# genome-vendor/bsmap

Measured on NVIDIA B200. Metric: wgbs_100nt_reads_mapped_per_sec, higher is better.
Workload: dtype u32

## Files before the change

### bsmap_b200/csrc/bsx_map_impl.cuh

```cuda
#include <type_traits>
#include "bsx_map.cuh"

#include "bsx_prep.cuh"

namespace {

constexpr int ROUND_HS = bsx_round_hs(MapKernel::pe, MapKernel::rrbs, MapKernel::wide);
constexpr int FW = MapKernel::wide ? 2 : 1;

enum { CT_CAND = 0, CT_PROBE, CT_OVER, CT_FULL, CT_COMMIT, CT_MAPPED, CT_LIST, CT_GATHER };
typedef uint32_t Ctr;
#define WSET(lhs, rhs) do { const auto v_ = (rhs); __syncwarp(); if (lane == 0) (lhs) = v_; __syncwarp(); } while (0)
#define CTR_ADD(C, k, v) do { const uint32_t v_ = (uint32_t)(v); if (lane == 0) (C)[k] += v_; } while (0)

__device__ __forceinline__ uint4 *plan_of(ReadSm *R, int chain, const MapArgs &A) {
    return reinterpret_cast<uint4 *>(reinterpret_cast<uint8_t *>(R) + sizeof(ReadSm)) + chain * A.chain_stride;
}
__device__ __forceinline__ uint4 *flank_of(ReadSm *R, int chain, const MapArgs &A) {
    return reinterpret_cast<uint4 *>(reinterpret_cast<uint8_t *>(R) + sizeof(ReadSm)) + A.flank_off + chain * A.chain_stride * FW;
}

__device__ __forceinline__ uint2 read_window(const ReadSm *R, int chain, int off) {
    if (off <= -16 || off >= 16 * BSX_FIXWORDS) return make_uint2(0u, 0u);
    if (off < 0) return make_uint2(R->rw[chain][0] >> (2 * -off), R->m5[chain][0] >> (2 * -off));
    const int j = off >> 4, sh = (off & 15) * 2;
    const uint32_t r1 = (j + 1 < BSX_FIXWORDS) ? R->rw[chain][j + 1] : 0u, m1 = (j + 1 < BSX_FIXWORDS) ? R->m5[chain][j + 1] : 0u;
    return make_uint2(__funnelshift_l(r1, R->rw[chain][j], sh), __funnelshift_l(m1, R->m5[chain][j], sh));
}

__device__ __forceinline__ uint32_t flank_mask(uint32_t q, uint32_t m5) { return m5 | ((m5 & ~(q & (q >> 1))) << 1); }
__device__ __forceinline__ uint32_t ctx_mm2(const uint4 f, const uint2 c) {
    const uint32_t ub = (f.x ^ c.x) & f.y, ua = (f.z ^ c.y) & f.w;
    return (uint32_t)__popc(((ub | (ub >> 1)) & 0x55555555u) | ((ua | (ua << 1)) & 0xAAAAAAAAu));
}

__device__ __forceinline__ void cp_async16s(uint32_t smem_addr, const void *gsrc) {
    asm volatile("cp.async.cg.shared.global.L2::64B [%0], [%1], 16;" :: "r"(smem_addr), "l"(gsrc) : "memory");
}
__device__ __forceinline__ void cp_async_commit() { asm volatile("cp.async.commit_group;" ::: "memory"); }
template <int N> __device__ __forceinline__ void cp_async_wait() { asm volatile("cp.async.wait_group %0;" :: "n"(N) : "memory"); }

__device__ __forceinline__ const CtaSm *cta_tables() {
    extern __shared__ __align__(16) uint8_t bsx_dyn_smem_[];
    return reinterpret_cast<const CtaSm *>(bsx_dyn_smem_);
}

__device__ __forceinline__ void init_cta_tables(const MapArgs &A, CtaSm *K) {
    #pragma unroll 1
    for (int t = threadIdx.x; t < 256; t += blockDim.x) K->profA[t] = (uint8_t)bsx_profile_a(A.s, A.I, t >> 4, t & 15);
    #pragma unroll 1
    for (int t = threadIdx.x; t < 160; t += blockDim.x) { K->segof[t] = (uint8_t)(t / A.s); K->remof[t] = (uint8_t)(t % A.s); }
    #pragma unroll 1
    for (int t = threadIdx.x; t < 258; t += blockDim.x) {
        int left = 0;
        if (t < 256 && A.n_seq < 65536u) {
            const uint32_t x = (uint32_t)t << 24;
            int right = (int)A.n_seq;
            while (left < right - 1) { const int mid = (left + right) / 2; if (x >= A.seqinfo[mid]) left = mid; else right = mid; }
        } else if (A.n_seq < 65536u) left = (int)A.n_seq - 1;
        K->chr_lut[t] = (uint16_t)left;
    }
    __syncthreads();
}

__device__ __forceinline__ void load_image(const MapArgs &A, ReadSm *R, const uint8_t *img, int lane) {
    __syncwarp();
    const uint4 hd = __ldcg(reinterpret_cast<const uint4 *>(img));
    const int len = (int)(hd.y & 0xffu), rmsn = (int)((hd.y >> 8) & 0xffu), seg = (int)((hd.y >> 16) & 0xffu);
    const int filtered = (int)((hd.y >> 24) & 1u), fc = (int)((hd.y >> 25) & 1u), cc = (int)((hd.y >> 26) & 1u);
    const int per = MapKernel::rrbs ? 1 : A.I, used = seg * per;
    if (!filtered) {
        #pragma unroll 1
        for (int c = 0; c < A.nslot; c++) {
            const int chain = A.nslot == 2 ? c : (fc ? 0 : 1);
            const uint8_t *sp = img + sizeof(ImgHdr) + (size_t)c * A.img_slot;
            if (lane < 2 * BSX_FIXWORDS) {
                const uint32_t v = __ldcg(reinterpret_cast<const uint32_t *>(sp) + lane);
                if (lane < BSX_FIXWORDS) R->rw[chain][lane] = v; else R->m5[chain][lane - BSX_FIXWORDS] = v;
            }
            uint4 *pl = plan_of(R, chain, A);
            const uint4 *src = reinterpret_cast<const uint4 *>(sp + 2 * BSX_FIXWORDS * 4);
            #pragma unroll 1
            for (int t = lane; t < used; t += 32) pl[t] = __ldcg(src + t);
        }
    }
    if (lane < 16) reinterpret_cast<uint32_t *>(R->nh)[lane] = 0u;
    if (lane == 0) {
        R->raw = (int)(hd.z & 0xffu); R->readset = (int)((hd.z >> 8) & 0xffu); R->seedseg = seg; R->filtered = filtered;
        R->index = hd.x; R->len = len; R->rmsn = rmsn; R->nw = (len + 15) >> 4;
        R->thres = (uint32_t)rmsn; R->fc = fc; R->cc = cc; R->dn = 0; R->best = 99;
    }
    __syncwarp();
    if (!filtered) {
        #pragma unroll 1
        for (int c = 0; c < A.nslot; c++) {
            const int chain = A.nslot == 2 ? c : (fc ? 0 : 1);
            const uint4 *pl = plan_of(R, chain, A);
            uint4 *fl = flank_of(R, chain, A);
            #pragma unroll 1
            for (int t = lane; t < used; t += 32) {
                const int p = (int)(pl[t].w & 0xffffu);
                const uint2 wb = read_window(R, chain, p - 16), wa = read_window(R, chain, p + A.s);
                fl[t * FW] = make_uint4(wb.x, flank_mask(wb.x, wb.y), wa.x, flank_mask(wa.x, wa.y));
                if constexpr (MapKernel::wide) {
                    const uint2 wb2 = read_window(R, chain, p - 32), wa2 = read_window(R, chain, p + A.s + 16);
                    fl[t * FW + 1] = make_uint4(wb2.x, flank_mask(wb2.x, wb2.y), wa2.x, flank_mask(wa2.x, wa2.y));
                }
            }
        }
    }
    __syncwarp();
}

__device__ __forceinline__ void prepare_block(const MapArgs &A, const CtaSm *K, PrepCol *P, uint8_t *scratch, uint32_t u0, uint32_t cnt, int lane, Ctr *C) {
    int np = 0;
    if ((uint32_t)lane < cnt) np = bsx_prep_unit(A, K, &P->rw[0][lane], &P->m5[0][lane], u0 + (uint32_t)lane, scratch + (size_t)lane * A.img_bytes);
#pragma unroll
    for (int d = 16; d; d >>= 1) np += __shfl_xor_sync(BSX_FULL, np, d);
    CTR_ADD(C, CT_PROBE, np);
    __syncwarp();
}

__device__ __forceinline__ uint32_t chunk_table(const ReadSm *R, int chain, int nw, int zlo, int zhi, int lane) {
    const int o = (lane / 3) & 3, dl = lane % 3;
    int score = 0;
    if (lane < 12) {
        const int jlo = 4 * dl - o;
#pragma unroll
        for (int t = 0; t < 3; t++) {
            const int j = jlo + t;
            if (j >= 0 && j < nw) {
                int lo = max(zlo, 16 * j) - 16 * j, hi = min(zhi, 16 * j + 16) - 16 * j;
                uint32_t seedm = 0;
                if (lo < hi) {
                    uint32_t a = 0xffffffffu >> (2 * lo);
                    uint32_t b = (hi >= 16) ? 0u : (0xffffffffu >> (2 * hi));
                    seedm = a & ~b;
                }
                score += __popc(R->m5[chain][j] & ~seedm);
            }
        }
    }
    const int oo = lane & 3;
    const int a0 = __shfl_sync(BSX_FULL, score, 3 * oo), a1 = __shfl_sync(BSX_FULL, score, 3 * oo + 1),
              a2 = __shfl_sync(BSX_FULL, score, 3 * oo + 2);
    int best = 0, bs = a0;
    if (a1 > bs) { best = 1; bs = a1; }
    if (a2 > bs) { best = 2; }
    uint32_t tb = (uint32_t)best << (2 * oo);
    return __shfl_sync(BSX_FULL, tb, 0) | __shfl_sync(BSX_FULL, tb, 1) | __shfl_sync(BSX_FULL, tb, 2) | __shfl_sync(BSX_FULL, tb, 3);
}

__device__ __forceinline__ uint32_t partial_mismatch(const ReadSm *R, int chain, int nw, const uint32_t *__restrict__ refbase,
                                                     uint32_t loc, uint32_t tbl) {
    const uint32_t wi = loc >> 4, sh2 = (loc & 15u) * 2u, o = wi & 3u;
    const uint32_t dl = (tbl >> (2 * o)) & 3u;
    const int jlo = 4 * (int)dl - (int)o;
    uint4 c;
    {
        const uint4 *gp = reinterpret_cast<const uint4 *>(refbase) + (wi >> 2) + dl;
        asm volatile("ld.global.nc.L2::64B.v4.u32 {%0,%1,%2,%3}, [%4];" : "=r"(c.x), "=r"(c.y), "=r"(c.z), "=r"(c.w) : "l"(gp));
    }
    uint32_t w = 0;
    int j = jlo;
    if (j >= 0 && j < nw) w += __popc(bsx_mm_word_bits(R->rw[chain][j], R->m5[chain][j], __funnelshift_l(c.y, c.x, sh2)));
    j++;
    if (j >= 0 && j < nw) w += __popc(bsx_mm_word_bits(R->rw[chain][j], R->m5[chain][j], __funnelshift_l(c.z, c.y, sh2)));
    j++;
    if (j >= 0 && j < nw) w += __popc(bsx_mm_word_bits(R->rw[chain][j], R->m5[chain][j], __funnelshift_l(c.w, c.z, sh2)));
    return w;
}

__device__ __forceinline__ uint32_t full_mismatch(const ReadSm *R, int chain, int nw, const uint32_t *__restrict__ refbase,
                                                  uint32_t loc, uint32_t thres) {
    const uint32_t *rp = refbase + (loc >> 4);
    const uint32_t sh2 = (loc & 15u) * 2u;
    uint32_t w = 0, prev = __ldg(rp);
    #pragma unroll 1
    for (int j = 0; j < nw; j++) {
        const uint32_t next = __ldg(rp + j + 1);
        w += __popc(bsx_mm_word_bits(R->rw[chain][j], R->m5[chain][j], __funnelshift_l(next, prev, sh2)));
        prev = next;
        if (w > thres) break;
    }
    return w;
}

__device__ int ccgg_seglen(const MapArgs &A, uint32_t chr, uint32_t pos, int readlen) {
    const uint32_t *st = A.sites + A.site_off[chr >> 1];
    const int n = (int)(A.site_off[(chr >> 1) + 1] - A.site_off[chr >> 1]);
    int left = 0, right = n - 1;
    while (left < right - 1) {
        int mid = (left + right) / 2;
        uint32_t mv = st[mid];
        if (mv == pos) { left = mid; right = mid + 1; break; }
        else if (mv < pos) left = mid; else right = mid;
    }
    const uint32_t seg_start = st[left], add = (uint32_t)(A.site_len - 2 * A.digest_pos);
    uint32_t seg_end;
    for (;;) {
        int rr = right < n ? right : n - 1;
        seg_end = st[rr] + add;
        if (seg_end < pos + (uint32_t)readlen && right < n) right++; else break;
    }
    return (int)(seg_end - seg_start);
}

__device__ int commit_hit(const MapArgs &A, ReadSm *R, uint2 *hits, uint32_t *dd, int store_all, int chain,
                          uint32_t chr, uint32_t loc, uint32_t w, int mode, int frag_filter, int lane, Ctr *C) {
    const uint32_t *anchor = A.seqinfo, *size = A.seqinfo + A.n_seq + 1, *rcoff = A.seqinfo + 2 * A.n_seq + 1;
    const uint32_t k = chr >> 1;
    if (chr & 1u) loc = rcoff[k] - (uint32_t)R->len - loc;
    if (loc + (uint32_t)R->len > size[k]) return 0;
    const uint32_t key = anchor[k] + loc;
    bool found = false;
    const uint32_t dn = R->dn;
    #pragma unroll 1
    for (uint32_t t = lane; t < dn; t += 32) found |= (dd[t] == key);
    if (__any_sync(BSX_FULL, found)) return 0;
    if (dn < A.dd_stride) {
        __syncwarp();
        if (lane == 0) { dd[dn] = key; R->dn = dn + 1; }
        __syncwarp();
    }
    if (frag_filter) {
        const int sl = ccgg_seglen(A, chr, loc, R->len);
        if (sl > A.max_insert || sl < A.min_insert) { __syncwarp(); return 0; }
    }
    if ((int)w < R->best) WSET(R->best, (int)w);
    if (lane == 0) {
        const uint32_t cnt = chain ? R->nc[w] : R->nh[w];
        if (store_all) hits[((size_t)w * 2 + chain) * (A.W + 1) + cnt] = make_uint2(chr, loc);
        else if ((int)w == R->best) hits[(size_t)chain * (A.W + 1) + cnt] = make_uint2(chr, loc);
        if (chain) R->nc[w] = (uint16_t)(cnt + 1); else R->nh[w] = (uint16_t)(cnt + 1);
    }
    __syncwarp();
    CTR_ADD(C, CT_COMMIT, 1);
    const int tot = (int)R->nh[w] + (int)R->nc[w];
    if ((int)w == mode && !A.pairend && A.r == 0 && tot > 1) return 1;
    if (tot >= A.W) { if (w == 0) return 1; WSET(R->thres, w - 1); }
    return 0;
}

__device__ __forceinline__ int extend_and_commit(const MapArgs &A, ReadSm *R, uint2 *hits, uint32_t *dd,
                                              int store_all, int chain, int mode, bool pass, uint32_t idx0, uint32_t md,
                                              uint32_t p, uint32_t tbl, int use_p1, int lane, Ctr *C) {
    const uint32_t *anchor = A.seqinfo;
    uint32_t strand = 0, loc = anchor[0], chr = 0;
    if (pass) {
        const uint32_t idx = idx0 + lane;
        uint32_t entry;
        asm volatile("ld.global.nc.L2::64B.u32 %0, [%1];" : "=r"(entry) : "l"(A.pos + idx));
        if constexpr (!MapKernel::rrbs) { strand = idx >= md; loc = entry - p; }
        else {
            chr = __ldg(A.tag + idx) & 0xffffu; strand = chr & 1u; loc = entry - p + anchor[chr >> 1];
            if (entry < p) pass = false;
        }
    }
    const uint32_t *refbase = strand ? A.crefcat : A.refcat;
    uint32_t w = 0xffffu;
    if (use_p1) {
        CTR_ADD(C, CT_GATHER, __popc(__ballot_sync(BSX_FULL, pass)));
        if (pass) {
            w = partial_mismatch(R, chain, R->nw, refbase, loc, tbl);
            pass = w <= R->thres;
        }
    }
    const unsigned pm1 = __ballot_sync(BSX_FULL, pass);
    unsigned pm = 0;
    if (pm1) {
        if (__popc(pm1) <= 4) {
            const int nw = R->nw, j = lane & 15, g = lane >> 4;
            unsigned left = pm1;
            #pragma unroll 1
            while (left) {
                const int s0 = __ffs(left) - 1; left &= left - 1;
                const int s1 = left ? __ffs(left) - 1 : -1; if (left) left &= left - 1;
                const int src = g ? s1 : s0;
                const uint32_t loc_g = __shfl_sync(BSX_FULL, loc, src < 0 ? 0 : src);
                const uint32_t strand_g = __shfl_sync(BSX_FULL, strand, src < 0 ? 0 : src);
                uint32_t wj = 0;
                if (src >= 0 && j < nw) {
                    const uint32_t *rp = (strand_g ? A.crefcat : A.refcat) + (loc_g >> 4) + j;
                    const uint32_t a = __ldg(rp), b = __ldg(rp + 1);
                    wj = __popc(bsx_mm_word_bits(R->rw[chain][j], R->m5[chain][j], __funnelshift_l(b, a, (loc_g & 15u) * 2u)));
                }
#pragma unroll
                for (int d = 8; d; d >>= 1) wj += __shfl_xor_sync(BSX_FULL, wj, d);
                const uint32_t w0 = __shfl_sync(BSX_FULL, wj, 0), w1 = __shfl_sync(BSX_FULL, wj, 16);
                if (lane == s0) w = w0;
                if (lane == s1) w = w1;
            }
            if (pass) pass = w <= R->thres;
        } else if (pass) {
            w = full_mismatch(R, chain, R->nw, refbase, loc, R->thres);
            pass = w <= R->thres;
        }
        pm = __ballot_sync(BSX_FULL, pass);
        CTR_ADD(C, CT_FULL, __popc(pm1));
    }
    int ret = 0, last = 31;
    while (pm) {
        const int src = __ffs(pm) - 1;
        pm &= pm - 1;
        const uint32_t w_s = __shfl_sync(BSX_FULL, w, src);
        if (w_s > R->thres) continue;
        uint32_t loc_s = __shfl_sync(BSX_FULL, loc, src);
        const uint32_t strand_s = __shfl_sync(BSX_FULL, strand, src);
        uint32_t chr_s;
        if constexpr (!MapKernel::rrbs) {
            int left = 0, right = (int)A.n_seq;
            if (A.n_seq < 65536u) { const CtaSm *K = cta_tables(); left = K->chr_lut[loc_s >> 24]; right = K->chr_lut[(loc_s >> 24) + 1] + 1; }
            while (left < right - 1) { int mid = (left + right) / 2; if (loc_s >= anchor[mid]) left = mid; else right = mid; }
            chr_s = (uint32_t)left * 2u + strand_s;
            loc_s -= anchor[left];
        } else {
            chr_s = __shfl_sync(BSX_FULL, chr, src);
            loc_s -= anchor[chr_s >> 1];
        }
        ret = commit_hit(A, R,  hits, dd, store_all, chain, chr_s, loc_s, w_s, mode,
                         MapKernel::rrbs && chain == 0 && !A.pairend, lane, C);
        if (ret) { last = src; break; }
    }
    return ret | (last << 8);
}

struct NarrowStep {
    uint4 d;
    uint4 f;
};
struct WideStep {
    uint4 d, f;
    uint4 f2;
};
typedef std::conditional_t<MapKernel::wide, uint4, uint2> CtxEntry;
typedef std::conditional_t<MapKernel::wide, WideStep, NarrowStep> HalfStep;
struct StageSm {
    CtxEntry slot[ROUND_HS * 32];
    HalfStep sched[ROUND_HS];
};
static_assert(ROUND_HS % 2 == 0 && ROUND_HS <= 32, "half-steps are evaluated in pairs; one lane describes one half-step");

__device__ __forceinline__ uint32_t ctx_count(const NarrowStep &h, const uint2 c) { return ctx_mm2(h.f, c); }
__device__ __forceinline__ uint32_t ctx_count(const WideStep &h, const uint4 c) {
    return ctx_mm2(h.f, make_uint2(c.y, c.z)) + ctx_mm2(h.f2, make_uint2(c.x, c.w));
}

__device__ __noinline__ void packed_exit(const uint4 *plan, int per, StageSm *S, uint32_t cur, uint32_t xl, int lane, Ctr *C) {
    const uint4 sc = S->sched[cur].d;
    uint32_t nk = 0;
    if (lane < per) { const uint4 el = plan[lane]; nk = el.z - el.x; }
    const uint32_t all = __reduce_add_sync(BSX_FULL, nk);
    const uint32_t before = __reduce_add_sync(BSX_FULL, (uint32_t)lane < sc.w ? nk : 0u);
    const uint32_t counted = before + (sc.x + xl - sc.y) + 1u;
    uint32_t extra = 0;
    if (lane < ROUND_HS && (uint32_t)lane >= cur) {
        const uint4 t = S->sched[lane].d;
        uint32_t lo_i = max(t.x, t.y);
        const uint32_t hi_i = min(t.x + 32u, t.y + t.z);
        if ((uint32_t)lane == cur) lo_i = max(lo_i, t.x + xl + 1u);
        extra = hi_i > lo_i ? hi_i - lo_i : 0u;
    }
    const uint32_t req = counted + __reduce_add_sync(BSX_FULL, extra);
    if (lane == 0) { C[CT_LIST] -= all - req; C[CT_OVER] += req - counted; }
}

__device__ __noinline__ uint32_t mode_chunk_table(const MapArgs &A, const ReadSm *R, int chain, const uint4 *plan, int per, int lane) {
    int zlo = 1000, zhi = -1;
    if (lane < per) { zlo = zhi = (int)(plan[lane].w & 0xffffu); }
#pragma unroll
    for (int d = 8; d; d >>= 1) { zlo = min(zlo, __shfl_xor_sync(BSX_FULL, zlo, d)); zhi = max(zhi, __shfl_xor_sync(BSX_FULL, zhi, d)); }
    zlo = __shfl_sync(BSX_FULL, zlo, 0); zhi = __shfl_sync(BSX_FULL, zhi, 0) + A.s;
    return chunk_table(R, chain, R->nw, zlo, zhi, lane);
}

template <class Step = HalfStep>
__device__ __forceinline__ int snp_align_packed(const MapArgs &A, ReadSm *R, uint2 *hits, uint32_t *dd, int store_all, int mode, int lane, Ctr *C, StageSm *S) {
    const int per = MapKernel::rrbs ? 1 : A.I;
    const int chain_lo = R->fc ? 0 : 1, chain_hi = R->cc ? 2 : 1;
    #pragma unroll 1
    for (int chain = chain_lo; chain < chain_hi; chain++) {
        const uint4 *plan = plan_of(R, chain, A) + mode * per, *flank = flank_of(R, chain, A) + mode * per * FW;
        uint4 e = make_uint4(0u, 0u, 0u, 0u);
        if (lane < per) e = plan[lane];
        const uint32_t n = e.z - e.x;
        uint32_t cum = n ? (n + (MapKernel::wide ? 0u : (e.x & 1u)) + 31u) >> 5 : 0u;
        const uint32_t my_hs = cum;
        #pragma unroll 1
        for (int d = 1; d < per; d <<= 1) { const uint32_t t = __shfl_up_sync(BSX_FULL, cum, d); if (lane >= d) cum += t; }
        const uint32_t total_hs = __shfl_sync(BSX_FULL, cum, per - 1);
        if (total_hs == 0) continue;
        CTR_ADD(C, CT_LIST, __reduce_add_sync(BSX_FULL, n));
        uint32_t thres = R->thres;
        uint32_t run_end = 0;
        #pragma unroll 1
        for (uint32_t h0 = 0; h0 < total_hs; h0 += ROUND_HS) {
            if (MapKernel::run_advance && h0 + ROUND_HS <= run_end) {
                Step h = S->sched[ROUND_HS - 1];
                __syncwarp();
                if (lane < ROUND_HS) { h.d.x += 32u * ((uint32_t)lane + 1u); S->sched[lane] = h; }
                __syncwarp();
            } else if constexpr (MapKernel::owner_sched) {
                const uint32_t first = cum - my_hs;
                if constexpr (MapKernel::run_advance) {
                    const uint32_t idx = h0 + ROUND_HS - 1u;
                    const unsigned own = __ballot_sync(BSX_FULL, lane < per && first <= idx && idx < cum);
                    const uint32_t ce = __shfl_sync(BSX_FULL, cum, own ? __ffs(own) - 1 : 0);
                    run_end = own ? ce : 0u;
                }
                __syncwarp();
                if (lane < ROUND_HS && h0 + (uint32_t)lane >= total_hs) S->sched[lane] = Step{};
                if (lane < per && my_hs) {
                    const uint32_t lo = max(first, h0), hi = min(cum, h0 + (uint32_t)ROUND_HS);
                    if (lo < hi) {
                        Step h;
                        h.f = flank[lane * FW];
                        if constexpr (MapKernel::wide) h.f2 = flank[lane * FW + 1];
                        h.d = make_uint4((MapKernel::wide ? e.x : (e.x & ~1u)) + 32u * (lo - first), e.x, n, (uint32_t)lane);
                        #pragma unroll 1
                        for (uint32_t t = lo; t < hi; t++) { S->sched[t - h0] = h; h.d.x += 32u; }
                    }
                }
                __syncwarp();
            } else {
                const uint32_t target = h0 + (uint32_t)lane;
                int k = 0; uint32_t first = 0;
                #pragma unroll 1
                for (int j = 0; j < per; j++) { const uint32_t c = __shfl_sync(BSX_FULL, cum, j); if (c <= target) { k = j + 1; first = c; } }
                if constexpr (MapKernel::run_advance) {
                    const int kk = __shfl_sync(BSX_FULL, k, ROUND_HS - 1);
                    const uint32_t ce = __shfl_sync(BSX_FULL, cum, kk & 15);
                    run_end = kk < per ? ce : 0u;
                }
                __syncwarp();
                if (lane < ROUND_HS) {
                    Step h{};
                    if (k < per) {
                        const uint4 ek = plan[k];
                        h.d = make_uint4((MapKernel::wide ? ek.x : (ek.x & ~1u)) + 32u * (target - first), ek.x, ek.z - ek.x, (uint32_t)k);
                        h.f = flank[k * FW];
                        if constexpr (MapKernel::wide) h.f2 = flank[k * FW + 1];
                    }
                    S->sched[lane] = h;
                }
                __syncwarp();
            }
            if constexpr (MapKernel::wide) {
                const char *ctx = reinterpret_cast<const char *>(A.ctx) + 16u * (uint32_t)lane;
                uint32_t sp = (uint32_t)__cvta_generic_to_shared(&S->slot[lane]);
                asm volatile("" : "+r"(sp), "+l"(ctx));
#pragma unroll
                for (uint32_t q = 0; q < ROUND_HS; q++) {
                    const uint4 sc = S->sched[q].d;
                    if (sc.x + (uint32_t)lane < sc.y + sc.z) cp_async16s(sp + 512u * q, ctx + (size_t)sc.x * 16u);
                }
            } else {
                const uint32_t half = (uint32_t)lane >> 4, pr = 2u * ((uint32_t)lane & 15u);
                const char *ctx = reinterpret_cast<const char *>(A.ctx) + 8u * pr;
                uint32_t sp = (uint32_t)__cvta_generic_to_shared(&S->slot[half * 32u + pr]);
                asm volatile("" : "+r"(sp), "+l"(ctx));
#pragma unroll
                for (uint32_t q = 0; q < ROUND_HS / 2; q++) {
                    const uint4 sc = S->sched[2u * q + half].d;
                    if (sc.x + pr < sc.y + sc.z) cp_async16s(sp + 512u * q, ctx + (size_t)sc.x * 8u);
                }
            }
            cp_async_commit();
            cp_async_wait<0>();
            __syncwarp();
            const uint32_t nst = min((uint32_t)ROUND_HS, total_hs - h0);
            #pragma unroll 1
            for (uint32_t hs = 0; hs < nst; hs += 2) {
                bool pass0 = ctx_count(S->sched[hs], S->slot[hs * 32u + lane]) <= thres;
                bool pass1 = ctx_count(S->sched[hs + 1], S->slot[hs * 32u + 32u + lane]) <= thres;
                if (!__any_sync(BSX_FULL, pass0 || pass1)) continue;
                const uint4 s0 = S->sched[hs].d, s1 = S->sched[hs + 1].d;
                pass0 &= (s0.x + (uint32_t)lane - s0.y) < s0.z;
                pass1 &= (s1.x + (uint32_t)lane - s1.y) < s1.z;
                const unsigned pm0 = __ballot_sync(BSX_FULL, pass0), pm1 = __ballot_sync(BSX_FULL, pass1);
                if (!(pm0 | pm1)) continue;
                const int use_p1 = __popc(pm0) + __popc(pm1) > 2;
                const uint32_t tbl = use_p1 ? mode_chunk_table(A, R, chain, plan, per, lane) : 0u;
                int ret = 0;
#pragma unroll 1
                for (int h = 0; h < 2; h++) {
                    if (h ? pm1 : pm0) {
                        const uint4 sc = h ? s1 : s0;
                        const uint4 ek = plan[sc.w];
                        const int rc = extend_and_commit(A, R, hits, dd, store_all, chain, mode, h ? pass1 : pass0, sc.x, ek.y, ek.w & 0xffffu, tbl, use_p1, lane, C);
                        if (rc & 1) { packed_exit(plan, per, S, hs + (uint32_t)h, (uint32_t)(rc >> 8), lane, C); ret = 1; break; }
                    }
                }
                if (ret) return 1;
                thres = R->thres;
            }
        }
    }
    return 0;
}

__device__ __forceinline__ void run_align(const MapArgs &A, ReadSm *R, uint2 *hits, uint32_t *dd, int store_all, int lane, Ctr *C, StageSm *stage) {
    #pragma unroll 1
    for (int m = 0; m < R->seedseg; m++) {
        snp_align_packed(A, R, hits, dd, store_all, m, lane, C, stage);
        if (!MapKernel::rrbs && R->best <= m) return;
    }
}

__device__ void write_record(const MapArgs &A, const ReadSm *R, const uint2 *hits, int store_all,
                             bsx_rec *out, uint16_t *cnt, int lane) {
    if (cnt && lane < 16) cnt[lane] = (!R->filtered && lane <= R->rmsn) ? (uint16_t)(R->nh[lane] + R->nc[lane]) : (uint16_t)0;
    if (lane != 0) return;
    bsx_rec o;
    o.loc = 0; o.chr = 0; o.nhits = 0; o.nm = 0; o.chain = 0; o.status = (uint8_t)R->filtered; o.len = (uint8_t)R->len;
    if (!R->filtered) {
        const int ii = R->best <= R->rmsn ? R->best : R->rmsn + 1;
        const int sum = ii <= R->rmsn ? R->nh[ii] + R->nc[ii] : 0;
        o.nm = (uint8_t)ii;
        if (sum > 0) {
            const int j = sum > 1 ? (int)(bsx_myrand(R->index, A.randseed) % (uint32_t)sum) : 0;
            const int nh = R->nh[ii];
            const int chain = j >= nh;
            const size_t lvl = store_all ? (size_t)ii * 2 : 0;
            const uint2 h = hits[(lvl + chain) * (A.W + 1) + (chain ? j - nh : j)];
            o.chr = h.x; o.loc = h.y; o.nhits = (uint32_t)sum; o.chain = (uint8_t)chain;
        }
    }
    *out = o;
}

__device__ __forceinline__ void flush_counters(const MapArgs &A, Ctr *C, int lane) {
    __syncwarp();
    if (lane < 8) { atomicAdd(A.stats + lane, (unsigned long long)(lane == CT_CAND ? C[CT_LIST] - C[CT_OVER] : C[lane])); }
    __syncwarp();
    if (lane < 8) C[lane] = 0;
    __syncwarp();
}

__device__ __forceinline__ void map_se(const MapArgs &A) {
    extern __shared__ __align__(16) uint8_t smem[];
    const int lane = threadIdx.x & 31, wid = threadIdx.x >> 5;
    CtaSm *K = reinterpret_cast<CtaSm *>(smem);
    init_cta_tables(A, K);
    uint8_t *base = smem + sizeof(CtaSm) + A.warp_smem_se * wid;
    ReadSm *R = reinterpret_cast<ReadSm *>(base);
    SelSm *X = reinterpret_cast<SelSm *>(base + A.read_smem);
    PrepCol *P = reinterpret_cast<PrepCol *>(base + A.read_smem + sizeof(SelSm));
    const uint32_t gw = blockIdx.x * (blockDim.x >> 5) + wid;
    uint2 *hits = A.hit_scratch + (size_t)gw * A.hit_stride;
    uint32_t *dd = A.dd_scratch + (size_t)gw * A.dd_stride;
    Ctr *C = X->ctr;
    if (lane < 8) C[lane] = 0;
    __syncwarp();
    uint8_t *scratch = A.prep + (size_t)gw * 32u * A.img_bytes;
    for (;;) {
        uint32_t r0 = 0;
        if (lane == 0) r0 = atomicAdd(A.work_counter, A.block_units);
        r0 = __shfl_sync(BSX_FULL, r0, 0);
        if (r0 >= A.n) break;
        const uint32_t cnt = min(A.block_units, A.n - r0);
        prepare_block(A, K, P, scratch, r0, cnt, lane, C);
        #pragma unroll 1
        for (uint32_t i = 0; i < cnt; i++) {
            const uint32_t r = r0 + i;
            if (C[CT_LIST] & 0x80000000u) flush_counters(A, C, lane);
            load_image(A, R, scratch + (size_t)i * A.img_bytes, lane);
            if (!R->filtered) run_align(A, R, hits, dd, 0, lane, C, reinterpret_cast<StageSm *>(P));
            __syncwarp();
            write_record(A, R,  hits, 0, A.out_a + r, A.cnt_a ? A.cnt_a + (size_t)r * 16 : nullptr, lane);
            if (!R->filtered && R->best <= R->rmsn) CTR_ADD(C, CT_MAPPED, 1);
            __syncwarp();
        }
    }
    flush_counters(A, C, lane);
}

struct PairHitDev { uint32_t a_chr, a_loc, b_chr, b_loc; int32_t insert; uint32_t meta;  uint32_t pad0, pad1; };

__device__ void sort_hits(uint2 *h, int n, int lane) {
    if (n < 2) return;
    bool dirty = true;
    while (dirty) {
        bool sw = false;
        #pragma unroll 1
        for (int phase = 0; phase < 2; phase++) {
            #pragma unroll 1
            for (int i = phase + 2 * lane; i + 1 < n; i += 64) {
                const uint2 a = h[i], b = h[i + 1];
                if (a.x > b.x || (a.x == b.x && a.y > b.y)) { h[i] = b; h[i + 1] = a; sw = true; }
            }
            __syncwarp();
        }
        dirty = __any_sync(BSX_FULL, sw);
    }
}

__device__ int get_pairs(const MapArgs &A, const ReadSm *Ra, const ReadSm *Rb,
                         const uint2 *ha_all, const uint2 *hb_all, PairHitDev *pairs, uint16_t *npairs, int na, int nb) {
    if (na > Ra->rmsn || nb > Rb->rmsn) return 0;
    const size_t W1 = (size_t)A.W + 1;
    uint16_t &cnt = npairs[na + nb];
    PairHitDev *bucket = pairs + (size_t)(na + nb) * W1;
    for (int dir = 0; dir < 2; dir++) {
        const uint2 *ha = ha_all + ((size_t)na * 2 + dir) * W1;
        const uint2 *hb = hb_all + ((size_t)nb * 2 + (1 - dir)) * W1;
        const int cnt_a = dir ? Ra->nc[na] : Ra->nh[na];
        const int cnt_b = dir ? Rb->nh[nb] : Rb->nc[nb];
        uint32_t chra = 0xffffffffu; int bstart = 0, bend = 0;
        #pragma unroll 1
        for (int i = 0; i < cnt_a; i++) {
            const uint2 x = ha[i];
            if (chra != x.x) {
                chra = x.x;
                for (bstart = bend; bstart < cnt_b; bstart++) if (hb[bstart].x >= chra) break;
                for (bend = bstart; bend < cnt_b; bend++) if (hb[bend].x > chra) break;
            }
            #pragma unroll 1
            for (int j = bstart; j < bend; j++) {
                const uint2 y = hb[j];
                const bool a_first = dir ? ((chra & 1u) != 0) : ((chra & 1u) == 0);
                uint32_t seg_start, seg_end;
                if (!a_first) { seg_start = y.y; seg_end = x.y + (uint32_t)Ra->len; }
                else { seg_start = x.y; seg_end = y.y + (uint32_t)Rb->len; }
                const int ins = (int)(seg_end - seg_start);
                if (ins >= A.min_insert && ins <= A.max_insert) {
                    PairHitDev ph;
                    ph.a_chr = x.x; ph.a_loc = x.y; ph.b_chr = y.x; ph.b_loc = y.y; ph.insert = ins;
                    ph.meta = (uint32_t)dir | ((uint32_t)na << 8) | ((uint32_t)nb << 16); ph.pad0 = ph.pad1 = 0;
                    bucket[cnt++] = ph;
                    if ((int)cnt >= A.W) return 1;
                }
            }
        }
    }
    return cnt > 0;
}

__device__ void write_unpaired(const MapArgs &A, const ReadSm *R, const uint2 *hits, bsx_rec *out, uint16_t *cnt, int lane) {
    if (cnt && lane < 16) cnt[lane] = (!R->filtered && lane <= R->rmsn) ? (uint16_t)(R->nh[lane] + R->nc[lane]) : (uint16_t)0;
    if (lane != 0) return;
    bsx_rec o;
    o.loc = 0; o.chr = 0; o.nhits = 0; o.nm = 0; o.chain = 0; o.status = (uint8_t)R->filtered; o.len = (uint8_t)R->len;
    if (!R->filtered) {
        int na, ma = 0, ra = 0;
        for (na = 0; na <= R->rmsn; na++) if ((ma = R->nh[na] + R->nc[na]) > 0) break;
        uint2 h = make_uint2(0, 0);
        if (ma) {
            if (ma > 1) ra = (int)(bsx_myrand(R->index, A.randseed) % (uint32_t)ma);
            const int nh = R->nh[na];
            h = (ra < nh) ? hits[((size_t)na * 2) * (A.W + 1) + ra] : hits[((size_t)na * 2 + 1) * (A.W + 1) + (ra - nh)];
        }
        na %= (R->rmsn + 1);
        o.chr = h.x; o.loc = h.y; o.nhits = (uint32_t)ma; o.nm = (uint8_t)na;
        o.chain = (uint8_t)(ra >= (int)R->nh[na]);
    }
    *out = o;
}
// ... 133 lines not shown
```

### bsmap_b200/csrc/bsx_map_pe.cu

```cuda
struct MapKernel {
    static constexpr bool pe = true, rrbs = false;
    static constexpr bool wide = false;
    static constexpr bool owner_sched = false, run_advance = false;
};
#include "bsx_map_impl.cuh"

namespace {
__global__ void __launch_bounds__(BSX_WARPS_PER_CTA * 32, 4) bsx_map_pe_wgbs_kernel(const __grid_constant__ MapArgs A) { map_pe(A); }
}
extern const void *const bsx_map_pe_wgbs = (const void *)bsx_map_pe_wgbs_kernel;
```

### bsmap_b200/csrc/bsx_map_pe_rrbs.cu

```cuda
struct MapKernel {
    static constexpr bool pe = true, rrbs = true, wide = false;
    static constexpr bool owner_sched = false;
    static constexpr bool run_advance = true;
};
#include "bsx_map_impl.cuh"

namespace {
__global__ void __launch_bounds__(BSX_WARPS_PER_CTA * 32, 4) bsx_map_pe_rrbs_kernel(const __grid_constant__ MapArgs A) { map_pe(A); }
}
extern const void *const bsx_map_pe_rrbs = (const void *)bsx_map_pe_rrbs_kernel;
```

### bsmap_b200/csrc/bsx_map_pe_wide.cu

```cuda
struct MapKernel {
    static constexpr bool pe = true, rrbs = false, wide = true;
    static constexpr bool owner_sched = false;
    static constexpr bool run_advance = true;
};
#include "bsx_map_impl.cuh"

namespace {
__global__ void __launch_bounds__(BSX_WARPS_PER_CTA * 32, 4) bsx_map_pe_wide_kernel(const __grid_constant__ MapArgs A) { map_pe(A); }
}
extern const void *const bsx_map_pe_wide = (const void *)bsx_map_pe_wide_kernel;
```

### bsmap_b200/csrc/bsx_map_se.cu

```cuda
struct MapKernel {
    static constexpr bool pe = false, rrbs = false, wide = false;
    static constexpr bool owner_sched = true;
    static constexpr bool run_advance = false;
};
#include "bsx_map_impl.cuh"

namespace {
__global__ void __launch_bounds__(BSX_WARPS_PER_CTA * 32, 5) bsx_map_se_wgbs_kernel(const __grid_constant__ MapArgs A) { map_se(A); }
}
extern const void *const bsx_map_se_wgbs = (const void *)bsx_map_se_wgbs_kernel;
```

### bsmap_b200/csrc/bsx_map_se_rrbs.cu

```cuda
struct MapKernel {
    static constexpr bool pe = false, rrbs = true, wide = false;
    static constexpr bool owner_sched = false;
    static constexpr bool run_advance = true;
};
#include "bsx_map_impl.cuh"

namespace {
__global__ void __launch_bounds__(BSX_WARPS_PER_CTA * 32, 5) bsx_map_se_rrbs_kernel(const __grid_constant__ MapArgs A) { map_se(A); }
}
extern const void *const bsx_map_se_rrbs = (const void *)bsx_map_se_rrbs_kernel;
```

### bsmap_b200/csrc/bsx_map_se_wide.cu

```cuda
struct MapKernel {
    static constexpr bool pe = false, rrbs = false, wide = true;
    static constexpr bool owner_sched = false;
    static constexpr bool run_advance = true;
};
#include "bsx_map_impl.cuh"

namespace {
__global__ void __launch_bounds__(BSX_WARPS_PER_CTA * 32, 5) bsx_map_se_wide_kernel(const __grid_constant__ MapArgs A) { map_se(A); }
}
extern const void *const bsx_map_se_wide = (const void *)bsx_map_se_wide_kernel;
```

### bsmap_b200/csrc/bsx_map.cuh

```cuda
#pragma once
#include "bsx_common.cuh"
#include "../../include/bsmap_b200.h"

#define BSX_MAX_KEYS 144
#define BSX_WARPS_PER_CTA 8
#define BSX_MAX_CTA_SMEM (227u * 1024u)

struct MapArgs {
    const uint32_t *refcat, *crefcat, *tab, *pos, *tag, *seqinfo;
    const void *ctx;
    int ctx_wide;
    const uint32_t *sites, *site_off;
    uint32_t n_seq;
    int s, I, v, W, r, min_insert, max_insert, chains, pairend, rrbs, randseed, max_ns, max_readlen;
    int n_adapter, site_len, digest_pos;
    uint32_t seed_bits;
    uint32_t rrbs_groups;
    int plan_cap;
    int nslot;
    uint32_t read_smem, warp_smem_se, chain_stride, flank_off;
    uint32_t img_slot, img_bytes;
    int adapter_len[BSX_MAX_ADAPTERS];
    char adapter[BSX_MAX_ADAPTERS][64];
    char digest_site[32];
    const uint8_t *seq_a, *seq_b;
    const uint16_t *len_a, *len_b;
    uint32_t stride, n, first_index;
    int readset;
    int packed;
    uint32_t pk_mask_off, pk_maxlen;
    bsx_rec *out_a, *out_b;
    bsx_pair_rec *out_pair;
    uint16_t *cnt_a, *cnt_b;
    uint32_t *work_counter;
    unsigned long long *stats;
    uint2 *hit_scratch;
    uint32_t *dd_scratch;
    uint4 *pair_scratch;
    uint32_t hit_stride, dd_stride, pair_stride;
    uint32_t *debug;
    uint8_t *prep;
    int mates;
    uint32_t block_units;
};

struct ImgHdr {
    uint32_t index;
    uint32_t geom;
    uint32_t aux;
    uint32_t pad;
};
static_assert(sizeof(ImgHdr) == 16, "image header is one uint4");

struct ReadSm {
    uint32_t rw[2][BSX_FIXWORDS];
    uint32_t m5[2][BSX_FIXWORDS];
    uint16_t nh[16], nc[16];
    int raw, seedseg, readset, filtered;
    uint32_t index;
    int len, rmsn, nw;
    uint32_t thres;
    int fc, cc;
    uint32_t dn;
    int best;
    uint32_t pad_[3];
};
static_assert(sizeof(ReadSm) % 16 == 0, "images are copied as uint4");

struct PrepCol {
    uint32_t rw[BSX_FIXWORDS][32], m5[BSX_FIXWORDS][32];
};

static_assert(sizeof(PrepCol) >= 4 * 32 * 16, "the align phase stages list heads (4 lists x 32 uint4) in the idle PrepCol");

struct SelSm {
    uint16_t npairs[32];
    uint32_t ctr[8];
};

struct CtaSm {
    uint8_t profA[16 * 16];
    uint8_t segof[160], remof[160];
    uint16_t chr_lut[264];
};
static_assert(sizeof(CtaSm) % 16 == 0, "per-warp shared memory follows CtaSm and holds uint4");

constexpr __host__ __device__ int bsx_round_hs(int pe, int , int wide) { return (pe && !wide) ? 12 : 8; }
static inline __host__ __device__ size_t bsx_stage_extra_bytes(int wide, int pe, int rrbs) {
    const size_t need = (size_t)bsx_round_hs(pe, rrbs, wide) * (wide ? 32u * 16u + 48u : 32u * 8u + 32u);
    return need > sizeof(PrepCol) ? ((need - sizeof(PrepCol) + 15u) & ~(size_t)15u) : 0u;
}
static inline __host__ __device__ size_t bsx_read_smem_bytes(int plan_cap, int nslot, int wide) {
    return sizeof(ReadSm) + (size_t)nslot * (size_t)plan_cap * (wide ? 3u : 2u) * sizeof(uint4);
}
static inline size_t bsx_warp_smem_bytes(int reads_per_warp, int plan_cap, int nslot, int wide, int rrbs) {
    return (size_t)reads_per_warp * bsx_read_smem_bytes(plan_cap, nslot, wide) + sizeof(SelSm) + sizeof(PrepCol) + bsx_stage_extra_bytes(wide, reads_per_warp == 2, rrbs);
}
static inline size_t bsx_cta_smem_bytes(int reads_per_warp, int plan_cap, int nslot, int wide, int rrbs, int warps) {
    return sizeof(CtaSm) + bsx_warp_smem_bytes(reads_per_warp, plan_cap, nslot, wide, rrbs) * (size_t)warps;
}

static inline void bsx_map_args_derive(MapArgs &a) {
    a.read_smem = (uint32_t)bsx_read_smem_bytes(a.plan_cap, a.nslot, a.ctx_wide);
    a.warp_smem_se = (uint32_t)bsx_warp_smem_bytes(1, a.plan_cap, a.nslot, a.ctx_wide, a.rrbs);
    a.chain_stride = a.nslot == 2 ? (uint32_t)a.plan_cap : 0u;
    a.flank_off = (uint32_t)(a.nslot * a.plan_cap);
    a.img_slot = (uint32_t)(2 * BSX_FIXWORDS * 4 + a.plan_cap * sizeof(uint4));
    a.img_bytes = (uint32_t)(sizeof(ImgHdr) + a.nslot * a.img_slot);
}
static inline size_t bsx_image_bytes(int plan_cap, int nslot) {
    return sizeof(ImgHdr) + (size_t)nslot * (2 * BSX_FIXWORDS * 4 + (size_t)plan_cap * sizeof(uint4));
}
```

Measured before the change: 356.4 million.

## Add dense flattened candidate walk for single-end WGBS mapping kernel

Adds a dense walk for the single-end WGBS kernel. It takes a prefix sum over the I sub-seed candidate lists, assigns lanes to flattened candidate indices three warps-widths at a time, and finds each lane's owning list with a carry-based count-down. It then loads 8-byte context entries and filters them before extension and commit. The aim is to remove lane idling and the per-list scheduling overhead of the packed walk, at the cost of more shuffles and more register pressure. Counters are adjusted on early exit to keep the statistics consistent.

```diff
diff --git a/bsmap_b200/csrc/bsx_map_impl.cuh b/bsmap_b200/csrc/bsx_map_impl.cuh
--- a/bsmap_b200/csrc/bsx_map_impl.cuh
+++ b/bsmap_b200/csrc/bsx_map_impl.cuh
@@ -7,6 +7,7 @@
 
 constexpr int ROUND_HS = bsx_round_hs(MapKernel::pe, MapKernel::rrbs, MapKernel::wide);
 constexpr int FW = MapKernel::wide ? 2 : 1;
+constexpr int DENSE_HALVES = 3;
 
 enum { CT_CAND = 0, CT_PROBE, CT_OVER, CT_FULL, CT_COMMIT, CT_MAPPED, CT_LIST, CT_GATHER };
 typedef uint32_t Ctr;
@@ -248,7 +249,7 @@
     const uint32_t *anchor = A.seqinfo;
     uint32_t strand = 0, loc = anchor[0], chr = 0;
     if (pass) {
-        const uint32_t idx = idx0 + lane;
+        const uint32_t idx = MapKernel::dense_walk ? idx0 : idx0 + lane;
         uint32_t entry;
         asm volatile("ld.global.nc.L2::64B.u32 %0, [%1];" : "=r"(entry) : "l"(A.pos + idx));
         if constexpr (!MapKernel::rrbs) { strand = idx >= md; loc = entry - p; }
@@ -499,10 +500,100 @@
     return 0;
 }
 
+__device__ __forceinline__ uint32_t count_down_if_below(uint32_t k, uint32_t q, uint32_t c) {
+    uint32_t r;
+    asm("{\n\t.reg .u32 t;\n\tsub.cc.u32 t, %1, %2;\n\tsubc.u32 %0, %3, 0;\n\t}" : "=r"(r) : "r"(q), "r"(c), "r"(k));
+    return r;
+}
+
+template <class T, int N> __device__ __forceinline__ T pick(const T (&a)[N], int h) {
+    T r = a[0];
+#pragma unroll
+    for (int i = 1; i < N; i++) if (h == i) r = a[i];
+    return r;
+}
+
+__device__ __forceinline__ void dense_exit(uint32_t total, uint32_t q0, int h, uint32_t xl, int lane, Ctr *C) {
+    const uint32_t counted = q0 + 32u * (uint32_t)h + xl + 1u, req = min(total, q0 + 32u * DENSE_HALVES);
+    if (lane == 0) { C[CT_LIST] -= total - req; C[CT_OVER] += req - counted; }
+}
+
+__device__ __forceinline__ int snp_align_dense(const MapArgs &A, ReadSm *R, uint2 *hits, uint32_t *dd, int store_all, int mode, int lane, Ctr *C) {
+    static_assert(!MapKernel::dense_walk || (!MapKernel::pe && !MapKernel::rrbs && !MapKernel::wide),
+                  "the dense walk serves the single-end WGBS kernel: 8-byte context entries, lists of the I sub-seeds");
+    constexpr int NH = DENSE_HALVES;
+    const int per = A.I;
+    const int chain_lo = R->fc ? 0 : 1, chain_hi = R->cc ? 2 : 1;
+    #pragma unroll 1
+    for (int chain = chain_lo; chain < chain_hi; chain++) {
+        const uint4 *plan = plan_of(R, chain, A) + mode * per, *flank = flank_of(R, chain, A) + mode * per;
+        uint32_t start = 0, n = 0;
+        if (lane < per) { const uint4 e = plan[lane]; start = e.x; n = e.z - e.x; }
+        uint32_t cum = n;
+        #pragma unroll 1
+        for (int d = 1; d < per; d <<= 1) { const uint32_t t = __shfl_up_sync(BSX_FULL, cum, d); if (lane >= d) cum += t; }
+        const uint32_t total = __shfl_sync(BSX_FULL, cum, per - 1);
+        if (total == 0) continue;
+        const uint32_t off = start - (cum - n);
+        if (lane >= per) cum = 0xffffffffu;
+        CTR_ADD(C, CT_LIST, total);
+        uint32_t thres = R->thres;
+        #pragma unroll 1
+        for (uint32_t q0 = 0; q0 < total; q0 += 32u * NH) {
+            uint32_t q[NH], k[NH], idx[NH];
+#pragma unroll
+            for (int h = 0; h < NH; h++) { q[h] = min(q0 + 32u * h + (uint32_t)lane, total - 1u); k[h] = (uint32_t)(per + 3) & ~3u; }
+            #pragma unroll 1
+            for (int j = 0; j < per; j += 4) {
+#pragma unroll
+                for (int u = 0; u < 4; u++) {
+                    const uint32_t c = __shfl_sync(BSX_FULL, cum, j + u);
+#pragma unroll
+                    for (int h = 0; h < NH; h++) k[h] = count_down_if_below(k[h], q[h], c);
+                }
+            }
+            uint2 ctx[NH];
+#pragma unroll
+            for (int h = 0; h < NH; h++) {
+                idx[h] = q[h] + __shfl_sync(BSX_FULL, off, k[h]);
+                asm volatile("ld.global.nc.L1::no_allocate.L2::64B.v2.u32 {%0,%1}, [%2];"
+                             : "=r"(ctx[h].x), "=r"(ctx[h].y) : "l"(reinterpret_cast<const uint2 *>(A.ctx) + idx[h]));
+            }
+            bool pass[NH], any = false;
+#pragma unroll
+            for (int h = 0; h < NH; h++) { pass[h] = ctx_mm2(flank[k[h]], ctx[h]) <= thres; any |= pass[h]; }
+            if (!__any_sync(BSX_FULL, any)) continue;
+            unsigned pm[NH];
+            int npass = 0;
+#pragma unroll
+            for (int h = 0; h < NH; h++) {
+                pass[h] &= q0 + 32u * h + (uint32_t)lane < total;
+                pm[h] = __ballot_sync(BSX_FULL, pass[h]); npass += __popc(pm[h]);
+            }
+            if (!npass) continue;
+            const int use_p1 = npass > 2;
+            const uint32_t tbl = use_p1 ? mode_chunk_table(A, R, chain, plan, per, lane) : 0u;
+            int ret = 0;
+#pragma unroll 1
+            for (int h = 0; h < NH; h++) {
+                if (pick(pm, h)) {
+                    const uint4 ek = plan[pick(k, h)];
+                    const int rc = extend_and_commit(A, R, hits, dd, store_all, chain, mode, pick(pass, h), pick(idx, h), ek.y, ek.w & 0xffffu, tbl, use_p1, lane, C);
+                    if (rc & 1) { dense_exit(total, q0, h, (uint32_t)(rc >> 8), lane, C); ret = 1; break; }
+                }
+            }
+            if (ret) return 1;
+            thres = R->thres;
+        }
+    }
+    return 0;
+}
+
 __device__ __forceinline__ void run_align(const MapArgs &A, ReadSm *R, uint2 *hits, uint32_t *dd, int store_all, int lane, Ctr *C, StageSm *stage) {
     #pragma unroll 1
     for (int m = 0; m < R->seedseg; m++) {
-        snp_align_packed(A, R, hits, dd, store_all, m, lane, C, stage);
+        if constexpr (MapKernel::dense_walk) snp_align_dense(A, R, hits, dd, store_all, m, lane, C);
+        else snp_align_packed(A, R, hits, dd, store_all, m, lane, C, stage);
         if (!MapKernel::rrbs && R->best <= m) return;
     }
 }
diff --git a/bsmap_b200/csrc/bsx_map_pe.cu b/bsmap_b200/csrc/bsx_map_pe.cu
--- a/bsmap_b200/csrc/bsx_map_pe.cu
+++ b/bsmap_b200/csrc/bsx_map_pe.cu
@@ -2,6 +2,7 @@
     static constexpr bool pe = true, rrbs = false;
     static constexpr bool wide = false;
     static constexpr bool owner_sched = false, run_advance = false;
+    static constexpr bool dense_walk = false;
 };
 #include "bsx_map_impl.cuh"
 
diff --git a/bsmap_b200/csrc/bsx_map_pe_rrbs.cu b/bsmap_b200/csrc/bsx_map_pe_rrbs.cu
--- a/bsmap_b200/csrc/bsx_map_pe_rrbs.cu
+++ b/bsmap_b200/csrc/bsx_map_pe_rrbs.cu
@@ -2,6 +2,7 @@
     static constexpr bool pe = true, rrbs = true, wide = false;
     static constexpr bool owner_sched = false;
     static constexpr bool run_advance = true;
+    static constexpr bool dense_walk = false;
 };
 #include "bsx_map_impl.cuh"
 
diff --git a/bsmap_b200/csrc/bsx_map_pe_wide.cu b/bsmap_b200/csrc/bsx_map_pe_wide.cu
--- a/bsmap_b200/csrc/bsx_map_pe_wide.cu
+++ b/bsmap_b200/csrc/bsx_map_pe_wide.cu
@@ -2,6 +2,7 @@
     static constexpr bool pe = true, rrbs = false, wide = true;
     static constexpr bool owner_sched = false;
     static constexpr bool run_advance = true;
+    static constexpr bool dense_walk = false;
 };
 #include "bsx_map_impl.cuh"
 
diff --git a/bsmap_b200/csrc/bsx_map_se.cu b/bsmap_b200/csrc/bsx_map_se.cu
--- a/bsmap_b200/csrc/bsx_map_se.cu
+++ b/bsmap_b200/csrc/bsx_map_se.cu
@@ -2,6 +2,7 @@
     static constexpr bool pe = false, rrbs = false, wide = false;
     static constexpr bool owner_sched = true;
     static constexpr bool run_advance = false;
+    static constexpr bool dense_walk = true;
 };
 #include "bsx_map_impl.cuh"
 
diff --git a/bsmap_b200/csrc/bsx_map_se_rrbs.cu b/bsmap_b200/csrc/bsx_map_se_rrbs.cu
--- a/bsmap_b200/csrc/bsx_map_se_rrbs.cu
+++ b/bsmap_b200/csrc/bsx_map_se_rrbs.cu
@@ -2,6 +2,7 @@
     static constexpr bool pe = false, rrbs = true, wide = false;
     static constexpr bool owner_sched = false;
     static constexpr bool run_advance = true;
+    static constexpr bool dense_walk = false;
 };
 #include "bsx_map_impl.cuh"
 
diff --git a/bsmap_b200/csrc/bsx_map_se_wide.cu b/bsmap_b200/csrc/bsx_map_se_wide.cu
--- a/bsmap_b200/csrc/bsx_map_se_wide.cu
+++ b/bsmap_b200/csrc/bsx_map_se_wide.cu
@@ -2,6 +2,7 @@
     static constexpr bool pe = false, rrbs = false, wide = true;
     static constexpr bool owner_sched = false;
     static constexpr bool run_advance = true;
+    static constexpr bool dense_walk = false;
 };
 #include "bsx_map_impl.cuh"
 
```

Measured after the change: 366.8 million (median of 6 runs). 1.03x the previous value.

## Use 16-candidate half-steps for narrow single-end non-RRBS seed scanning

Applied to the files above, without the earlier changes.

Adds a compile-time half-step width (HSE) that drops from 32 to 16 candidates in the narrow single-end non-RRBS configuration, and doubles the number of half-steps per staging round so the staged volume stays the same. Each warp-wide pass then evaluates four 16-candidate steps, with lanes mapped to sub-steps. The goal is less padding waste on short candidate runs, since each plan entry rounds up to 16 instead of 32. In exchange the schedule fill, the lane-to-candidate index maths and the early-exit accounting become more complex, and there are more schedule entries to write per round.

```diff
diff --git a/bsmap_b200/csrc/bsx_map.cuh b/bsmap_b200/csrc/bsx_map.cuh
--- a/bsmap_b200/csrc/bsx_map.cuh
+++ b/bsmap_b200/csrc/bsx_map.cuh
@@ -85,9 +85,10 @@
 };
 static_assert(sizeof(CtaSm) % 16 == 0, "per-warp shared memory follows CtaSm and holds uint4");
 
-constexpr __host__ __device__ int bsx_round_hs(int pe, int , int wide) { return (pe && !wide) ? 12 : 8; }
+constexpr __host__ __device__ int bsx_hs_entries(int pe, int rrbs, int wide) { return (!pe && !rrbs && !wide) ? 16 : 32; }
+constexpr __host__ __device__ int bsx_round_hs(int pe, int rrbs, int wide) { return (pe && !wide) ? 12 : 256 / bsx_hs_entries(pe, rrbs, wide); }
 static inline __host__ __device__ size_t bsx_stage_extra_bytes(int wide, int pe, int rrbs) {
-    const size_t need = (size_t)bsx_round_hs(pe, rrbs, wide) * (wide ? 32u * 16u + 48u : 32u * 8u + 32u);
+    const size_t need = (size_t)bsx_round_hs(pe, rrbs, wide) * (wide ? 32u * 16u + 48u : (size_t)bsx_hs_entries(pe, rrbs, wide) * 8u + 32u);
     return need > sizeof(PrepCol) ? ((need - sizeof(PrepCol) + 15u) & ~(size_t)15u) : 0u;
 }
 static inline __host__ __device__ size_t bsx_read_smem_bytes(int plan_cap, int nslot, int wide) {
diff --git a/bsmap_b200/csrc/bsx_map_impl.cuh b/bsmap_b200/csrc/bsx_map_impl.cuh
--- a/bsmap_b200/csrc/bsx_map_impl.cuh
+++ b/bsmap_b200/csrc/bsx_map_impl.cuh
@@ -6,6 +6,7 @@
 namespace {
 
 constexpr int ROUND_HS = bsx_round_hs(MapKernel::pe, MapKernel::rrbs, MapKernel::wide);
+constexpr uint32_t HSE = bsx_hs_entries(MapKernel::pe, MapKernel::rrbs, MapKernel::wide);
 constexpr int FW = MapKernel::wide ? 2 : 1;
 
 enum { CT_CAND = 0, CT_PROBE, CT_OVER, CT_FULL, CT_COMMIT, CT_MAPPED, CT_LIST, CT_GATHER };
@@ -336,10 +337,10 @@
 typedef std::conditional_t<MapKernel::wide, uint4, uint2> CtxEntry;
 typedef std::conditional_t<MapKernel::wide, WideStep, NarrowStep> HalfStep;
 struct StageSm {
-    CtxEntry slot[ROUND_HS * 32];
+    CtxEntry slot[ROUND_HS * HSE];
     HalfStep sched[ROUND_HS];
 };
-static_assert(ROUND_HS % 2 == 0 && ROUND_HS <= 32, "half-steps are evaluated in pairs; one lane describes one half-step");
+static_assert(ROUND_HS % (64 / HSE) == 0 && ROUND_HS <= 32, "a round holds whole 64-candidate steps; one lane describes one half-step");
 
 __device__ __forceinline__ uint32_t ctx_count(const NarrowStep &h, const uint2 c) { return ctx_mm2(h.f, c); }
 __device__ __forceinline__ uint32_t ctx_count(const WideStep &h, const uint4 c) {
@@ -357,7 +358,7 @@
     if (lane < ROUND_HS && (uint32_t)lane >= cur) {
         const uint4 t = S->sched[lane].d;
         uint32_t lo_i = max(t.x, t.y);
-        const uint32_t hi_i = min(t.x + 32u, t.y + t.z);
+        const uint32_t hi_i = min(t.x + HSE, t.y + t.z);
         if ((uint32_t)lane == cur) lo_i = max(lo_i, t.x + xl + 1u);
         extra = hi_i > lo_i ? hi_i - lo_i : 0u;
     }
@@ -384,7 +385,7 @@
         uint4 e = make_uint4(0u, 0u, 0u, 0u);
         if (lane < per) e = plan[lane];
         const uint32_t n = e.z - e.x;
-        uint32_t cum = n ? (n + (MapKernel::wide ? 0u : (e.x & 1u)) + 31u) >> 5 : 0u;
+        uint32_t cum = n ? (n + (MapKernel::wide ? 0u : (e.x & 1u)) + HSE - 1u) / HSE : 0u;
         const uint32_t my_hs = cum;
         #pragma unroll 1
         for (int d = 1; d < per; d <<= 1) { const uint32_t t = __shfl_up_sync(BSX_FULL, cum, d); if (lane >= d) cum += t; }
@@ -398,7 +399,7 @@
             if (MapKernel::run_advance && h0 + ROUND_HS <= run_end) {
                 Step h = S->sched[ROUND_HS - 1];
                 __syncwarp();
-                if (lane < ROUND_HS) { h.d.x += 32u * ((uint32_t)lane + 1u); S->sched[lane] = h; }
+                if (lane < ROUND_HS) { h.d.x += HSE * ((uint32_t)lane + 1u); S->sched[lane] = h; }
                 __syncwarp();
             } else if constexpr (MapKernel::owner_sched) {
                 const uint32_t first = cum - my_hs;
@@ -416,9 +417,9 @@
                         Step h;
                         h.f = flank[lane * FW];
                         if constexpr (MapKernel::wide) h.f2 = flank[lane * FW + 1];
-                        h.d = make_uint4((MapKernel::wide ? e.x : (e.x & ~1u)) + 32u * (lo - first), e.x, n, (uint32_t)lane);
+                        h.d = make_uint4((MapKernel::wide ? e.x : (e.x & ~1u)) + HSE * (lo - first), e.x, n, (uint32_t)lane);
                         #pragma unroll 1
-                        for (uint32_t t = lo; t < hi; t++) { S->sched[t - h0] = h; h.d.x += 32u; }
+                        for (uint32_t t = lo; t < hi; t++) { S->sched[t - h0] = h; h.d.x += HSE; }
                     }
                 }
                 __syncwarp();
@@ -437,7 +438,7 @@
                     Step h{};
                     if (k < per) {
                         const uint4 ek = plan[k];
-                        h.d = make_uint4((MapKernel::wide ? ek.x : (ek.x & ~1u)) + 32u * (target - first), ek.x, ek.z - ek.x, (uint32_t)k);
+                        h.d = make_uint4((MapKernel::wide ? ek.x : (ek.x & ~1u)) + HSE * (target - first), ek.x, ek.z - ek.x, (uint32_t)k);
                         h.f = flank[k * FW];
                         if constexpr (MapKernel::wide) h.f2 = flank[k * FW + 1];
                     }
@@ -455,28 +456,31 @@
                     if (sc.x + (uint32_t)lane < sc.y + sc.z) cp_async16s(sp + 512u * q, ctx + (size_t)sc.x * 16u);
                 }
             } else {
-                const uint32_t half = (uint32_t)lane >> 4, pr = 2u * ((uint32_t)lane & 15u);
+                constexpr uint32_t LPH = HSE / 2;
+                const uint32_t grp = (uint32_t)lane / LPH, pr = 2u * ((uint32_t)lane % LPH);
                 const char *ctx = reinterpret_cast<const char *>(A.ctx) + 8u * pr;
-                uint32_t sp = (uint32_t)__cvta_generic_to_shared(&S->slot[half * 32u + pr]);
+                uint32_t sp = (uint32_t)__cvta_generic_to_shared(&S->slot[grp * HSE + pr]);
                 asm volatile("" : "+r"(sp), "+l"(ctx));
 #pragma unroll
-                for (uint32_t q = 0; q < ROUND_HS / 2; q++) {
-                    const uint4 sc = S->sched[2u * q + half].d;
+                for (uint32_t q = 0; q < ROUND_HS * HSE / 64u; q++) {
+                    const uint4 sc = S->sched[(32u / LPH) * q + grp].d;
                     if (sc.x + pr < sc.y + sc.z) cp_async16s(sp + 512u * q, ctx + (size_t)sc.x * 8u);
                 }
             }
             cp_async_commit();
             cp_async_wait<0>();
             __syncwarp();
-            const uint32_t nst = min((uint32_t)ROUND_HS, total_hs - h0);
-            #pragma unroll 1
-            for (uint32_t hs = 0; hs < nst; hs += 2) {
-                bool pass0 = ctx_count(S->sched[hs], S->slot[hs * 32u + lane]) <= thres;
-                bool pass1 = ctx_count(S->sched[hs + 1], S->slot[hs * 32u + 32u + lane]) <= thres;
+            constexpr uint32_t SPS = 64u / HSE;
+            const uint32_t nst = min((uint32_t)ROUND_HS, total_hs - h0), xi = HSE == 32u ? (uint32_t)lane : (uint32_t)lane % HSE;
+            #pragma unroll 1
+            for (uint32_t hs = 0; hs < nst; hs += SPS) {
+                const uint32_t q = hs + (HSE == 32u ? 0u : (uint32_t)lane / HSE);
+                bool pass0 = ctx_count(S->sched[q], S->slot[hs * HSE + lane]) <= thres && (HSE == 32u || q < nst);
+                bool pass1 = ctx_count(S->sched[q + SPS / 2], S->slot[hs * HSE + 32u + lane]) <= thres && (HSE == 32u || q + SPS / 2 < nst);
                 if (!__any_sync(BSX_FULL, pass0 || pass1)) continue;
-                const uint4 s0 = S->sched[hs].d, s1 = S->sched[hs + 1].d;
-                pass0 &= (s0.x + (uint32_t)lane - s0.y) < s0.z;
-                pass1 &= (s1.x + (uint32_t)lane - s1.y) < s1.z;
+                const uint4 s0 = S->sched[q].d, s1 = S->sched[q + SPS / 2].d;
+                pass0 &= (s0.x + xi - s0.y) < s0.z;
+                pass1 &= (s1.x + xi - s1.y) < s1.z;
                 const unsigned pm0 = __ballot_sync(BSX_FULL, pass0), pm1 = __ballot_sync(BSX_FULL, pass1);
                 if (!(pm0 | pm1)) continue;
                 const int use_p1 = __popc(pm0) + __popc(pm1) > 2;
@@ -487,8 +491,12 @@
                     if (h ? pm1 : pm0) {
                         const uint4 sc = h ? s1 : s0;
                         const uint4 ek = plan[sc.w];
-                        const int rc = extend_and_commit(A, R, hits, dd, store_all, chain, mode, h ? pass1 : pass0, sc.x, ek.y, ek.w & 0xffffu, tbl, use_p1, lane, C);
-                        if (rc & 1) { packed_exit(plan, per, S, hs + (uint32_t)h, (uint32_t)(rc >> 8), lane, C); ret = 1; break; }
+                        const int rc = extend_and_commit(A, R, hits, dd, store_all, chain, mode, h ? pass1 : pass0, sc.x + xi - (uint32_t)lane, ek.y, ek.w & 0xffffu, tbl, use_p1, lane, C);
+                        if (rc & 1) {
+                            const uint32_t xl = (uint32_t)(rc >> 8);
+                            packed_exit(plan, per, S, hs + (uint32_t)h * (SPS / 2) + (HSE == 32u ? 0u : xl / HSE), HSE == 32u ? xl : xl % HSE, lane, C);
+                            ret = 1; break;
+                        }
                     }
                 }
                 if (ret) return 1;
```

Result: no change. 351.6 million before, 348.9 million after, median of 6 (-0.8%).
